# aksiksi/needle

Hardware: AMD Instinct MI355X
Metric: episode-pairs/sec (analyze+search) (higher is better)
Workload: dtype f64-certified (f32 first pass)

## Files before the change

include/needle_hip.h:

```cpp
#ifndef NEEDLE_HIP_H
#define NEEDLE_HIP_H

#include "needle.h"

#ifdef __cplusplus
extern "C" {
#endif

enum NeedleError needle_hip_device_count(int *count);
enum NeedleError needle_hip_set_device(int ordinal);
enum NeedleError needle_hip_synchronize(void);
enum NeedleError needle_hip_device_pci_bus_id(char out[32]);
void *needle_hip_stream(void);
const char *needle_hip_last_error_message(void);
const char *needle_hip_version(void);

enum NeedleError needle_hip_malloc(void **device_ptr, size_t bytes);
enum NeedleError needle_hip_free(void *device_ptr);
enum NeedleError needle_hip_memcpy_h2d(void *device_dst, const void *host_src, size_t bytes);
enum NeedleError needle_hip_memcpy_d2h(void *host_dst, const void *device_src, size_t bytes);
void needle_hip_host_free(void *ptr);
enum NeedleError needle_hip_host_alloc(void **host_ptr, size_t bytes);
enum NeedleError needle_hip_host_alloc_free(void *host_ptr);

double needle_hip_last_kernel_ms(const char *kernel);
void needle_hip_set_kernel_timing(const char *kernels);
enum NeedleError needle_hip_int_valu_ceiling(double *cells_per_second);
enum NeedleError needle_hip_scan_issued_evaluations(uint64_t *lane_evaluations, bool reset);
enum NeedleError needle_hip_scan_counts(uint64_t counts[2], bool reset);
enum NeedleError needle_hip_scan_last_launch(int32_t *form, uint64_t *matrix_products);
enum NeedleError needle_hip_epilogue_host_fallbacks(uint64_t *jobs, bool reset);

#define NEEDLE_HIP_MAX_CHANNELS 8
int needle_hip_fingerprint_sample_rate(void);
int needle_hip_fingerprint_delay_ms(void);
int needle_hip_fingerprint_item_duration_ms(void);
size_t needle_hip_fingerprint_num_items(size_t samples_per_channel);
size_t needle_hip_fingerprint_num_kept(size_t samples_per_channel, uint32_t step);

enum NeedleError needle_hip_fingerprint_host(const int16_t *const *pcm, const size_t *num_values,
                                             size_t num_streams, int channels, uint32_t step,
                                             uint32_t *const *items);

enum NeedleError needle_hip_fingerprint_device(const int16_t *d_pcm, const uint64_t *pcm_offsets,
                                               const uint64_t *num_values, size_t num_streams,
                                               int channels, uint32_t step, uint32_t *d_items,
                                               const uint64_t *item_offsets, bool sync);

enum NeedleError needle_hip_fingerprint_cert_stats(uint64_t counts[4], bool reset);

typedef struct NeedleHipCertAudit {
  uint64_t items, accepted, accepted_mismatches, mismatches;
  double max_error_over_s, max_s;
// ... 238 lines not shown
```

needle_amd/capi.py:

```python
from __future__ import annotations

import ctypes as C
import os
from dataclasses import dataclass
from typing import List, Optional, Sequence, Tuple

import numpy as np

NS = 1_000_000_000
LIB_PATH = os.environ.get("NEEDLE_CAPI_LIB") or os.path.join(os.path.dirname(os.path.abspath(__file__)), "lib", "libneedle_capi.so")

ERROR_NAMES = ["Ok", "InvalidUtf8String", "NullArgument", "InvalidArgument", "FrameHashDataNotFound",
               "FrameHashDataInvalidVersion", "InvalidFrameHashData", "ComparatorMinimumPaths",
               "AnalyzerInvalidHashPeriod", "AnalyzerInvalidHashDuration", "IOError", "Unknown"]

DEFAULT_HASH_MATCH_THRESHOLD = 10
DEFAULT_OPENING_SEARCH_PERCENTAGE = 0.50
DEFAULT_ENDING_SEARCH_PERCENTAGE = 0.25
DEFAULT_MIN_OPENING_DURATION = 20
DEFAULT_MIN_ENDING_DURATION = 20
DEFAULT_HASH_DURATION = 0.3
MAX_CHANNELS = 8


# ... 42 lines not shown
    "needle_hip_fingerprint_delay_ms", "needle_hip_fingerprint_item_duration_ms", "needle_hip_fingerprint_num_items",
    "needle_hip_fingerprint_num_kept", "needle_hip_fingerprint_host", "needle_hip_fingerprint_device",
    "needle_hip_fingerprint_debug", "needle_hip_resample_out_len", "needle_hip_resample_host", "needle_hip_downmix_host",
    "needle_hip_hamming_runs_device", "needle_hip_hamming_runs_host",
    "needle_hip_frame_hashes_new", "needle_hip_frame_hashes_free", "needle_hip_frame_hashes_len",
    "needle_hip_frame_hashes_copy", "needle_hip_frame_hashes_hash_duration_ns", "needle_hip_frame_hashes_md5",
    "needle_hip_frame_hashes_read", "needle_hip_frame_hashes_write", "needle_hip_header_md5",
    "needle_hip_analyzer_run_pcm", "needle_hip_comparator_run_with_frame_hashes", "needle_hip_library_new",
    "needle_hip_library_free", "needle_hip_library_include_endings", "needle_hip_library_set_sample_rate",
    "needle_hip_library_rows_per_video",
    "needle_hip_library_set_pcm", "needle_hip_library_set_pcm_device", "needle_hip_library_rank_videos",
    "needle_hip_library_analyze",
    "needle_hip_library_hash_arena", "needle_hip_library_use_hash_arena", "needle_hip_library_num_pairs", "needle_hip_library_search",
    "needle_hip_library_fetch_runs_begin", "needle_hip_library_fetch_runs_end",
    "needle_hip_library_finalize", "needle_hip_library_frame_hashes",
    "needle_hip_comm_create_id", "needle_hip_comm_init", "needle_hip_comm_finalize", "needle_hip_comm_rank",
    "needle_hip_comm_world_size", "needle_hip_comm_backend", "needle_hip_comm_barrier",
    "needle_hip_comm_all_gather_host", "needle_hip_comm_shard", "needle_hip_library_job_begin",
    "needle_hip_library_job_end", "needle_hip_library_stream_pcm", "needle_hip_host_alloc",
    "needle_hip_host_alloc_free", "needle_hip_int_valu_ceiling",
    "needle_hip_comparator_results_from_runs", "needle_hip_library_job_runs", "needle_hip_library_job_comm_bytes",
    "needle_hip_library_job_form",
    "needle_hip_host_threads", "needle_hip_fingerprint_audit_device", "needle_hip_library_audit",
    "needle_hip_scan_counts", "needle_hip_scan_last_launch", "needle_hip_epilogue_host_fallbacks",
    "needle_hip_index_new", "needle_hip_index_free", "needle_hip_index_len", "needle_hip_index_add",
    "needle_hip_index_results", "needle_hip_index_pairs_searched", "needle_hip_index_remove", "needle_hip_index_replace",
    "needle_hip_index_store_sizes", "needle_hip_index_crossmatcher_new", "needle_hip_index_add_matched",
    "needle_hip_index_pairs_scanned",
    "needle_hip_convert_host", "needle_hip_analyzer_run_pcm_format", "needle_hip_library_set_sample_format",
    "needle_hip_feeder_new", "needle_hip_feeder_free", "needle_hip_feeder_feed", "needle_hip_feeder_finish",
    "needle_hip_feeder_reset", "needle_hip_feeder_ready", "needle_hip_feeder_items", "needle_hip_feeder_frame_hashes",
    "needle_hip_feeder_state_bytes", "needle_hip_feeder_num_ready", "needle_hip_feeder_set_audit", "needle_hip_feeder_audit",
    "needle_hip_matcher_new", "needle_hip_matcher_free", "needle_hip_matcher_feed", "needle_hip_matcher_feed_from_feeder",
    "needle_hip_matcher_finish", "needle_hip_matcher_reset", "needle_hip_matcher_ready", "needle_hip_matcher_runs",
    "needle_hip_matcher_open", "needle_hip_matcher_stats",
    "needle_hip_crossmatcher_new", "needle_hip_crossmatcher_free", "needle_hip_crossmatcher_feed",
    "needle_hip_crossmatcher_feed_from_feeder", "needle_hip_crossmatcher_finish", "needle_hip_crossmatcher_ready",
    "needle_hip_crossmatcher_lane", "needle_hip_crossmatcher_runs", "needle_hip_crossmatcher_stats",
    "needle_hip_crossmatcher_state_bytes", "needle_hip_crossmatcher_new_regions",
    "needle_hip_crossmatcher_state_bytes_regions", "needle_hip_crossmatcher_shape",
    "needle_hip_crossmatcher_new_resident", "needle_hip_crossmatcher_state_bytes_resident", "needle_hip_crossmatcher_resident"]

SAMPLE_U8, SAMPLE_S16, SAMPLE_S32, SAMPLE_F32, SAMPLE_F64 = 0, 1, 2, 3, 4
SAMPLE_U8P, SAMPLE_S16P, SAMPLE_S32P, SAMPLE_F32P, SAMPLE_F64P = 5, 6, 7, 8, 9
_SAMPLE_DTYPES = [np.uint8, np.int16, np.int32, np.float32, np.float64]


# ... 246 lines not shown


def scan_issued_evaluations(reset: bool = False) -> int:
    v = C.c_uint64(0)
    lib().needle_hip_scan_issued_evaluations.argtypes = [C.POINTER(C.c_uint64), C.c_bool]
    check(lib().needle_hip_scan_issued_evaluations(C.byref(v), reset))
    return int(v.value)


def scan_counts(reset: bool = False) -> Tuple[int, int]:
    c = (C.c_uint64 * 2)()
    lib().needle_hip_scan_counts.argtypes = [C.POINTER(C.c_uint64), C.c_bool]
    check(lib().needle_hip_scan_counts(c, reset))
    return int(c[0]), int(c[1])


def scan_last_launch() -> Tuple[int, int]:
    form, products = C.c_int32(0), C.c_uint64(0)
    lib().needle_hip_scan_last_launch.argtypes = [C.POINTER(C.c_int32), C.POINTER(C.c_uint64)]
    check(lib().needle_hip_scan_last_launch(C.byref(form), C.byref(products)))
    return int(form.value), int(products.value)


def epilogue_host_fallbacks(reset: bool = False) -> int:
    jobs = C.c_uint64(0)
    lib().needle_hip_epilogue_host_fallbacks.argtypes = [C.POINTER(C.c_uint64), C.c_bool]
    check(lib().needle_hip_epilogue_host_fallbacks(C.byref(jobs), reset))
    return int(jobs.value)


def host_threads() -> int:
    lib().needle_hip_host_threads.restype = C.c_int
    return int(lib().needle_hip_host_threads())


def int_valu_ceiling() -> float:
    v = C.c_double(0.0)
    lib().needle_hip_int_valu_ceiling.argtypes = [C.POINTER(C.c_double)]
    check(lib().needle_hip_int_valu_ceiling(C.byref(v)))
    return v.value


def last_kernel_ms(name: str) -> float:
    return lib().needle_hip_last_kernel_ms(name.encode())


# ... 925 lines not shown
```

needle_amd/csrc/capi.cpp:

```cpp
#include <dirent.h>
#include <hip/hip_runtime_api.h>
#include <sys/stat.h>

#include <algorithm>
#include <cstdio>
#include <cstdlib>
#include <chrono>
#include <cstring>
#include <fstream>
#include <new>

#include "crossmatch.h"
#include "epilogue.h"
#include "hipctx.h"
#include "feeder.h"
#include "index.h"
#include "matcher.h"
#include "needle_core.h"

using namespace needle;

struct FrameHashes {
  FrameHashesData d;
};
// ... 409 lines not shown

enum NeedleError needle_hip_scan_issued_evaluations(uint64_t *lane_evaluations, bool reset) {
  if (!lane_evaluations) return NeedleError_NullArgument;
  return guarded([&]() -> NeedleError {
    Status s = gpu_scan_issued_evaluations(lane_evaluations, reset);
    return s.ok() ? NeedleError_Ok : report(s);
  });
}

enum NeedleError needle_hip_scan_counts(uint64_t counts[2], bool reset) {
  if (!counts) return NeedleError_NullArgument;
  return guarded([&]() -> NeedleError {
    Status s = gpu_scan_issued_evaluations(&counts[0], reset, &counts[1]);
    return s.ok() ? NeedleError_Ok : report(s);
  });
}

enum NeedleError needle_hip_scan_last_launch(int32_t *form, uint64_t *matrix_products) {
  if (!form || !matrix_products) return NeedleError_NullArgument;
  gpu_scan_last_launch(form, matrix_products);
  return NeedleError_Ok;
}

enum NeedleError needle_hip_epilogue_host_fallbacks(uint64_t *jobs, bool reset) {
  if (!jobs) return NeedleError_NullArgument;
  *jobs = reset ? epilogue_host_fallbacks().exchange(0) : epilogue_host_fallbacks().load();
  return NeedleError_Ok;
}

enum NeedleError needle_hip_int_valu_ceiling(double *cells_per_second) {
  if (!cells_per_second) return NeedleError_NullArgument;
  return guarded([&]() -> NeedleError {
    Status s = gpu_int_valu_ceiling(cells_per_second);
    return s.ok() ? NeedleError_Ok : report(s);
  });
}

double needle_hip_last_kernel_ms(const char *kernel) { return kernel ? kernel_ms(kernel) : -1.0; }
void needle_hip_set_kernel_timing(const char *kernels) { set_kernel_timing(kernels); }

int needle_hip_fingerprint_sample_rate(void) { return kSampleRate; }
int needle_hip_fingerprint_delay_ms(void) { return kDelayMs; }
int needle_hip_fingerprint_item_duration_ms(void) { return kItemDurationMs; }
size_t needle_hip_fingerprint_num_items(size_t samples_per_channel) { return num_items(samples_per_channel); }
size_t needle_hip_fingerprint_num_kept(size_t samples_per_channel, uint32_t step) {
  return num_kept(samples_per_channel, step);
// ... 771 lines not shown
```

needle_amd/csrc/common.h:

```cpp
#pragma once

#include <cstddef>
#include <cstdint>
#include <functional>
#include <string>
#include <vector>

#include "../../include/needle_hip.h"

struct ihipStream_t;

namespace needle {

struct Status {
  NeedleError code = NeedleError_Ok;
  std::string message;
  bool ok() const { return code == NeedleError_Ok; }
  static Status Ok() { return Status{}; }
  static Status Make(NeedleError c, std::string m) { return Status{c, std::move(m)}; }
};

NeedleError report(const Status &s);
void set_last_error(const std::string &m);
const char *last_error();
// ... 80 lines not shown
                              uint32_t step, uint32_t *d_items, bool sync, double *d_chroma_dbg = nullptr,
                              double *d_feat_dbg = nullptr, size_t descriptor_slot = 0, int pipe = -1,
                              uint32_t *zero_word = nullptr, bool *zeroed = nullptr);
Status gpu_fingerprint_streamed_device(const std::vector<const int16_t *> &pcm, const std::vector<size_t> &num_values,
                                       int channels, uint32_t step, uint32_t *d_items,
                                       const std::vector<uint64_t> &item_off, int rate = kSampleRate);
Status gpu_fingerprint_host(const std::vector<const int16_t *> &pcm, const std::vector<size_t> &num_values,
                            int channels, uint32_t step, std::vector<std::vector<uint32_t>> *items,
                            int rate = kSampleRate);
using PcmReader = std::function<Status(size_t stream, uint64_t first_value, uint64_t num_values, int16_t *dst)>;
using StreamIssued = std::function<Status(size_t stream_index)>;
Status gpu_upload_pcm_streamed(const std::vector<size_t> &num_values, const std::vector<uint64_t> &dev_off,
                               const PcmReader &read, unsigned readers, int16_t *d_pcm, ::ihipStream_t *stream = nullptr,
                               const StreamIssued &issued = nullptr);
Status gpu_upload_pcm(const std::vector<const int16_t *> &pcm, const std::vector<size_t> &num_values,
                      const std::vector<uint64_t> &dev_off, int16_t *d_pcm, ::ihipStream_t *stream = nullptr,
                      const StreamIssued &issued = nullptr);
Status gpu_fingerprint_streamed(const std::vector<size_t> &num_values, const PcmReader &read, unsigned readers,
                                int channels, uint32_t step, std::vector<std::vector<uint32_t>> *items,
                                int rate = kSampleRate);
Status gpu_hamming_runs_device(const uint32_t *d_hashes, const NeedleHipSeq *seqs, size_t num_seqs,
                               const NeedleHipProblem *problems, size_t num_problems, uint32_t threshold,
                               NeedleHipRun *d_runs, uint32_t capacity, uint32_t *d_count, bool sync,
                               bool count_is_zero = false);
Status gpu_hamming_runs_host(const uint32_t *hashes, size_t num_hashes, const NeedleHipSeq *seqs, size_t num_seqs,
                             const NeedleHipProblem *problems, size_t num_problems, uint32_t threshold,
                             std::vector<NeedleHipRun> *runs);

uint32_t *gpu_pinned_arena_acquire(size_t words);
void gpu_pinned_arena_release(uint32_t *arena);
void gpu_prefetch_hashes(const uint32_t *hashes, size_t num_hashes);

constexpr uint64_t kDeviceEpiloguePairs = 1u << 14;
constexpr uint32_t kDeviceEpilogueRuns = 1u << 14;

Status gpu_int_valu_ceiling(double *cells_per_second);
Status gpu_scan_issued_evaluations(uint64_t *lane_evaluations, bool reset, uint64_t *head_survivors = nullptr);
void gpu_scan_last_launch(int32_t *form, uint64_t *matrix_products);
Status gpu_fingerprint_cert_stats(uint64_t out[4], bool reset);
Status gpu_fingerprint_audit_device(const int16_t *d_pcm, const std::vector<StreamSpan> &spans, int channels, uint32_t step,
                                    const uint32_t *d_items, uint64_t out[4], double *max_ratio, double *max_sigma);

struct FeedLane {
  uint64_t pcm_off;
  uint64_t item_off;
  uint32_t row_base;
  uint32_t carried;
  uint32_t frames;
  uint32_t first_item;
  uint32_t kept;
  uint32_t lane;
};
constexpr size_t kFeedAuditWords = 6;
struct FeedAudit {
  double *rows64;
  uint64_t *counts;
};
Status gpu_fingerprint_feed_device(const int16_t *d_pcm, const std::vector<FeedLane> &lanes, int channels, uint32_t step,
                                   double *d_chroma, float *d_energy, double *d_chroma64, uint32_t *d_items,
                                   const FeedAudit *audit = nullptr);
bool gpu_fingerprint_f64_mode();
// ... 57 lines not shown
```

needle_amd/csrc/library.cpp:

```cpp
#include <hip/hip_runtime_api.h>

#include <algorithm>
#include <chrono>
#include <cstdio>
#include <cstdlib>
#include <cstring>
#include <map>
#include <new>
#include <tuple>

#include "comm.h"
#include "epilogue.h"
#include "hipctx.h"
#include "needle_core.h"

struct FrameHashes;
struct NeedleAudioComparator;

namespace needle {
const Comparator &comparator_of(const NeedleAudioComparator *c);
FrameHashes *make_frame_hashes(FrameHashesData &&d);
void fill_c_result(const VideoResult &v, NeedleHipSearchResult *r);
}

// ... 729 lines not shown
      if (num_pairs) pair_at(lib->n, first_pair, &i, &j);
      for (size_t p = first_pair; p < first_pair + num_pairs; p++) {
        for (size_t r = 0; r < Rc; r++) {
          if (r == 1 && (lib->win[i * R + 1].kept == 0 || lib->win[j * R + 1].kept == 0))
            return report(Status::Make(NeedleError_Unknown, "no ending hash data present"));
          const uint32_t a = lib->min_len[i * R + r], b = lib->min_len[j * R + r];
          if (a == 0 || b == 0) continue;
          problems.push_back(NeedleHipProblem{(uint32_t)(i * R + r), (uint32_t)(j * R + r), std::max(a, b),
                                              (uint32_t)(p * Rc + r)});
        }
        if (++j == lib->n) j = ++i + 1;
      }
      lib->problems_for[0] = first_pair;
      lib->problems_for[1] = num_pairs;
      lib->problems_for[2] = Rc;
    }
    for (NeedleHipLibrary::Fetch &f : lib->fetch)
      if (f.pending && (f.d_runs == d_runs || f.d_count == d_count) &&
          hipStreamWaitEvent(library_stream(), f.done, 0) != hipSuccess)
        return report(Status::Make(NeedleError_Unknown, "stream wait failed"));
    const auto t_built = std::chrono::steady_clock::now();
    const bool count_is_zero = lib->count_zeroed == d_count;
    lib->count_zeroed = nullptr;
    Status s = gpu_hamming_runs_device(lib->arena, seqs.data(), seqs.size(), problems.data(), problems.size(),
                                       cmp.hash_match_threshold(), d_runs, capacity, d_count, sync, count_is_zero);
    if (getenv("NEEDLE_HIP_TRACE"))
      std::fprintf(stderr, "[needle_hip] search enqueue: %zu problems built in %.2f ms, launched in %.2f ms\n",
                   problems.size(), std::chrono::duration<double, std::milli>(t_built - t_enter).count(),
                   std::chrono::duration<double, std::milli>(std::chrono::steady_clock::now() - t_built).count());
    return s.ok() ? NeedleError_Ok : report(s);
  });
}

enum NeedleError needle_hip_library_fetch_runs_begin(NeedleHipLibrary *lib, int slot, const NeedleHipRun *d_runs,
                                                     const uint32_t *d_count, uint32_t max_runs) {
  if (!lib || !d_runs || !d_count) return NeedleError_NullArgument;
  if (slot < 0 || slot > 1 || max_runs == 0) return NeedleError_InvalidArgument;
  return guarded([&]() -> NeedleError {
    NeedleHipLibrary::Fetch &f = lib->fetch[slot];
    if (f.pending) return report(Status::Make(NeedleError_InvalidArgument, "fetch slot still pending"));
    const size_t bytes = 16 + (size_t)max_runs * sizeof(NeedleHipRun);
    if (f.max_runs < max_runs) {
      if (f.host) (void)hipHostFree(f.host);
      f.host = nullptr;
      if (hipHostMalloc(&f.host, bytes, hipHostMallocDefault) != hipSuccess)
        return report(Status::Make(NeedleError_Unknown, "pinned allocation failed"));
      f.max_runs = max_runs;
    }
// ... 736 lines not shown
```

needle_amd/csrc/search.hip:

```cpp
#include "epilogue.h"
#include "hipctx.h"
#include "simhash_wave.h"

#include <algorithm>
#include <atomic>
#include <cstdio>
#include <cstdlib>
#include <cstring>
#include <mutex>
#include <unordered_map>

namespace needle {

namespace {

constexpr int kDiagsPerBlock = 256;
constexpr int kBandR = 7, kBandU = 3;
constexpr int kBandB = 64 * kBandR;
constexpr int kSampleW = 8;
constexpr int kSampleHead = 3;
__host__ __device__ constexpr int head_row(int k, int W, int H = kSampleHead) {
  return H == 3 ? (k == 0 ? 0 : (k == 1 ? W / 2 : W - 1)) : (k * (W - 1)) / (H - 1);
}
__host__ __device__ constexpr bool is_head_row(int s, int W, int H = kSampleHead) {
// ... 158 lines not shown
#pragma unroll
    for (int r = 0; r < R; r++) any |= (i + K - 1 - Z[r] >= flag_len);
    if (__any(any)) checkpoint(i + K - 1);
  }
  for (; i <= i_end; i++) {
    const uint32_t sv = src[i];
#pragma unroll
    for (int r = 0; r < R; r++) {
      const uint32_t c = (uint32_t)__popc(sv ^ W[r]);
      Z[r] = (c <= threshold) ? Z[r] : i;
    }
#pragma unroll
    for (int r = 0; r + 1 < R; r++) W[r] = W[r + 1];
    W[R - 1] = lds[B + i + d_l + R];
  }
}

__device__ __forceinline__ void wave_lds_fence_search() {
  __builtin_amdgcn_fence(__ATOMIC_RELEASE, "wavefront");
  __builtin_amdgcn_wave_barrier();
  __builtin_amdgcn_fence(__ATOMIC_ACQUIRE, "wavefront");
}

template <int R, int W, bool COUNT = false, int H = kSampleHead, bool LEGACY = false>
__global__ __launch_bounds__(256) void hamming_runs_sampled_kernel(const uint32_t *__restrict__ hashes,
                                                                   const SearchProblem *__restrict__ problems,
                                                                   int num_problems, uint32_t threshold,
                                                                   NeedleHipRun *__restrict__ runs,
                                                                   uint32_t capacity, uint32_t *__restrict__ count,
                                                                   int bands_per_wave, int sparse_max,
                                                                   unsigned long long *__restrict__ eval_groups) {
  constexpr int B = 64 * R;
  unsigned long long groups = 0, survived = 0;
  extern __shared__ uint32_t lds[];
  __builtin_amdgcn_s_setprio(3);
  int lo = 0, hi = num_problems - 1;
  while (lo < hi) {
    int mid = (lo + hi + 1) >> 1;
    if (problems[mid].block_base <= blockIdx.x) lo = mid; else hi = mid - 1;
  }
  const SearchProblem pr = problems[lo];
  const int n = (int)pr.n, m = (int)pr.m;
  const uint32_t *__restrict__ src = hashes + pr.src_off;
  const uint32_t *__restrict__ dst = hashes + pr.dst_off;
  uint32_t *ldst = lds;
  for (int k = threadIdx.x; k < B; k += blockDim.x) {
    ldst[k] = 0u;
    ldst[B + m + k] = 0u;
  }
  {
    constexpr int kU = 8;
    const int nt = (int)blockDim.x;
    int k = threadIdx.x;
    for (; k + (kU - 1) * nt < m; k += kU * nt) {
// ... 46 lines not shown

  int k0 = (i_start - 1 + P - 1) / P;
  for (int w0 = 1 + k0 * P; w0 + W - 1 <= i_end; w0 += P) {
    uint32_t E[W + R - 1];
#pragma unroll
    for (int q = 0; q < W + R - 1; q++) E[q] = ldst[B + w0 + d_l + q];
    uint32_t sv[W];
#pragma unroll
    for (int s = 0; s < W; s++) sv[s] = src[w0 + s];
    bool ok[R];
    uint32_t miss[R];
#pragma unroll
    for (int r = 0; r < R; r++) miss[r] = 0u;
#pragma unroll
    for (int k = 0; k < H; k++) {
      const int s = head_row(k, W, H);
#pragma unroll
      for (int r = 0; r < R; r++) miss[r] |= (uint32_t)__popc(sv[s] ^ E[s + r]) + bias;
    }
#pragma unroll
    for (int r = 0; r < R; r++) ok[r] = miss[r] < 32u;
    if (COUNT) groups += H * R;
    auto resolve = [&](const int d) {
      const int ilo = d < 0 ? 1 - d : 1;
      const int ihi = min(n - 1, m - 1 - d);
      if (w0 < ilo || w0 + W - 1 > ihi) return;
      int e = w0 + W;
      bool ended = false;
      const int fwd_limit = min(ihi, w0 + P + W - 1);
      while (e <= fwd_limit) {
        const int row = e + lane;
        const bool bad = row <= fwd_limit && (uint32_t)__popc(lsrc[row] ^ ldst[B + row + d]) > threshold;
        if (COUNT) groups += 1;
        const unsigned long long mm = __ballot(bad);
        if (mm) {
          e += __ffsll((long long)mm) - 1;
          ended = true;
          break;
        }
        e += 64;
      }
      if (!ended) {
        if (fwd_limit == w0 + P + W - 1) return;
        e = ihi + 1;
      }
      const int b = e - 1;
      int a = ilo;
      int q = w0 - 1;
      while (q >= ilo) {
        const int row = q - lane;
        const bool bad = row >= ilo && (uint32_t)__popc(lsrc[row] ^ ldst[B + row + d]) > threshold;
        if (COUNT) groups += 1;
        const unsigned long long mm = __ballot(bad);
        if (mm) {
          a = q - (__ffsll((long long)mm) - 1) + 1;
          break;
        }
        q -= 64;
      }
      const int len = b - a + 1;
      if (len >= min_len) emit_run((uint32_t)b, (uint32_t)(b + d), (uint32_t)len);
    };

    unsigned long long alive[R];
    int survivors = 0;
#pragma unroll
    for (int r = 0; r < R; r++) {
      alive[r] = __ballot(ok[r]);
      survivors += __popcll(alive[r]);
    }
    if (COUNT) survived += (unsigned long long)survivors;
    if (survivors == 0) continue;
    if (!LEGACY || sparse_max < 0) {
#pragma unroll
      for (int r = 0; r < R; r++) {
        if (alive[r] == 0) continue;
        uint32_t mm = miss[r];
#pragma unroll
        for (int k = 0; k < W - H; k++) {
          const int s = tail_row(k, W, H);
          mm |= (uint32_t)__popc(sv[s] ^ E[s + r]) + bias;
        }
        if (COUNT) groups += W - H;
        unsigned long long cand = __ballot(mm < 32u);
        while (cand) {
          const int src_lane = __ffsll((long long)cand) - 1;
          cand &= cand - 1;
          resolve(D0 + src_lane * R + r);
        }
      }
      continue;
    }
    if constexpr (LEGACY) {
    if (survivors <= sparse_max) {
      constexpr int kTail = W - H;
      uint32_t sv_tail = sv[tail_row(kTail - 1, W, H)];
      int tail_off = tail_row(kTail - 1, W, H);
#pragma unroll
      for (int k = kTail - 2; k >= 0; k--) {
        sv_tail = lane == k ? sv[tail_row(k, W, H)] : sv_tail;
        tail_off = lane == k ? tail_row(k, W, H) : tail_off;
      }
#pragma unroll
      for (int r = 0; r < R; r++) {
        unsigned long long cand = alive[r];
        while (cand) {
          const int src_lane = __ffsll((long long)cand) - 1;
// ... 13 lines not shown
#pragma unroll
      for (int r = 0; r < R; r++) miss[r] |= (uint32_t)__popc(sv[s] ^ E[s + r]) + bias;
    }
#pragma unroll
    for (int r = 0; r < R; r++) ok[r] = miss[r] < 32u;
    if (COUNT) groups += (W - H) * R;
#pragma unroll
    for (int r = 0; r < R; r++) {
      unsigned long long cand = __ballot(ok[r]);
      while (cand) {
        const int src_lane = __ffsll((long long)cand) - 1;
        cand &= cand - 1;
        resolve(D0 + src_lane * R + r);
      }
    }
    }
  }
  }
  flush_runs();
  if (COUNT && lane == 0) {
    atomicAdd(eval_groups, groups);
    atomicAdd(eval_groups + 1, survived);
  }
}

__host__ __device__ constexpr int mfma_windows(int n, int min_len, int W) {
  return (n - 1 - W) >= 0 && min_len - W + 1 > 0 ? (n - 1 - W) / (min_len - W + 1) + 1 : 0;
}
typedef int mfma_v4i __attribute__((ext_vector_type(4)));
typedef int mfma_v8i __attribute__((ext_vector_type(8)));
typedef float mfma_v16f __attribute__((ext_vector_type(16)));

#include "scan_mfma_kernel.h"


__global__ __launch_bounds__(256) void simhash_runs_kernel(const uint32_t *__restrict__ hashes,
                                                           const SearchProblem *__restrict__ problems,
                                                           NeedleHipRun *__restrict__ runs, uint32_t capacity,
                                                           const uint32_t *__restrict__ count) {
  const uint32_t total = min(*count, capacity);
  const uint32_t wave = (blockIdx.x * blockDim.x + threadIdx.x) >> 6, waves = (gridDim.x * blockDim.x) >> 6;
  const uint32_t lane = threadIdx.x & 63;
  __builtin_amdgcn_s_setprio(3);
  const TransposeLane t = transpose_lane(lane);
  for (uint32_t k = wave; k < total; k += waves) {
    const NeedleHipRun r = runs[k];
// ... 3 lines not shown
    if (lane == 0) {
      runs[k].problem = pr.tag;
      runs[k].src_match_hash = src_hash;
      runs[k].dst_match_hash = dst_hash;
    }
  }
}

struct ScanShape {
  int w = kSampleW, h = kSampleHead;
};
ScanShape scan_shape() {
  ScanShape sh;
  if (const char *e = getenv("NEEDLE_HIP_SCAN_SHAPE")) {
    int w = 0, h = 0;
    if (std::sscanf(e, "%d,%d", &w, &h) == 2 && (w == 4 || w == 8 || w == 16) && h >= 2 && h <= 4 && h < w) {
      sh.w = w;
      sh.h = h;
    }
  }
  return sh;
}
using SampledKernel = void (*)(const uint32_t *, const SearchProblem *, int, uint32_t, NeedleHipRun *, uint32_t, uint32_t *, int, int,
                               unsigned long long *);
template <bool COUNT>
SampledKernel sampled_kernel(ScanShape sh, bool legacy) {
#define NEEDLE_SHAPE(W_, H_) \
  if (sh.w == W_ && sh.h == H_) return hamming_runs_sampled_kernel<kBandR, W_, COUNT, H_, true>;
  NEEDLE_SHAPE(4, 2) NEEDLE_SHAPE(4, 3) NEEDLE_SHAPE(8, 2) NEEDLE_SHAPE(8, 4) NEEDLE_SHAPE(16, 2) NEEDLE_SHAPE(16, 3) NEEDLE_SHAPE(16, 4)
#undef NEEDLE_SHAPE
  if (legacy) return hamming_runs_sampled_kernel<kBandR, kSampleW, COUNT, kSampleHead, true>;
  return hamming_runs_sampled_kernel<kBandR, kSampleW, COUNT, kSampleHead, false>;
}

struct SearchPlan {
  std::vector<NeedleHipSeq> seqs;
  std::vector<NeedleHipProblem> problems;
  int mode[8] = {0, 0, 0, 0, 0, 0, 0, 0};
  std::vector<SearchProblem> meta;
  size_t staged = 0;
  uint64_t oversize_blocks = 0;
  uint64_t blocks = 0;
  size_t lds_bytes = 0;
  bool sampled = false, fast = false, mfma = false;
  int mfma_waves = 0, mfma_splits = 1;
  std::vector<M2ImageSeq> image_seqs;
  uint32_t image_windows = 0, image_min_len = 0;
// ... 217 lines not shown
}

int mfma_request(uint32_t threshold) {
  if (threshold > 15u || scan_shape().w != kSampleW || getenv("NEEDLE_HIP_SCAN_SHAPE") || getenv("NEEDLE_HIP_SCAN_COUNT")) return 0;
  const char *e = getenv("NEEDLE_HIP_SCAN_MFMA");
  if (!e) return 2;
  return atoi(e) != 0 ? 1 : 0;
}

int mfma_waves() {
  int waves = 8;
  if (const char *e = getenv("NEEDLE_HIP_MFMA_WAVES")) {
    const int w = atoi(e);
    if (w == 4 || w == 8 || w == 12 || w == 16) waves = w;
  }
  return waves;
}
using Mfma2Kernel = void (*)(const uint32_t *, const SearchProblem *, int, uint32_t, NeedleHipRun *, uint32_t, uint32_t *, int, const uint32_t *);
Mfma2Kernel mfma2_kernel(int waves) {
  return waves == 4 ? hamming_runs_mfma2_kernel<kSampleW, 4, 3> : waves == 16 ? hamming_runs_mfma2_kernel<kSampleW, 16, 4>
       : waves == 12 ? hamming_runs_mfma2_kernel<kSampleW, 12, 3> : hamming_runs_mfma2_kernel<kSampleW, 8, 4>;
}

std::atomic<int32_t> g_last_form{0};
std::atomic<uint64_t> g_last_products{0};

struct SearchWorkspace {
  DeviceBuffer<SearchProblem> problems;
  PinnedStage stage;
  DescriptorUpload<SearchProblem> upload;
  SearchPlan plan;
  DeviceBuffer<M2ImageSeq> image_seqs;
  PinnedStage image_stage;
  DescriptorUpload<M2ImageSeq> image_upload;
  DeviceBuffer<uint32_t> images;
  bool lds_attr_set = false;
  unsigned long long *eval_groups = nullptr;
};
std::mutex g_ws_mu;
std::map<int, SearchWorkspace *> g_ws;

SearchWorkspace *workspace() {
  int dev = 0;
  (void)hipGetDevice(&dev);
  std::lock_guard<std::mutex> lock(g_ws_mu);
  auto it = g_ws.find(dev);
  if (it != g_ws.end()) return it->second;
  SearchWorkspace *w = new SearchWorkspace();
  g_ws[dev] = w;
  return w;
}


}

void gpu_scan_last_launch(int32_t *form, uint64_t *matrix_products) {
  *form = g_last_form.load();
  *matrix_products = g_last_products.load();
}

Status gpu_hamming_runs_device(const uint32_t *d_hashes, const NeedleHipSeq *seqs, size_t num_seqs,
                               const NeedleHipProblem *problems, size_t num_problems, uint32_t threshold,
                               NeedleHipRun *d_runs, uint32_t capacity, uint32_t *d_count, bool sync, bool count_is_zero) {
  std::lock_guard<std::recursive_mutex> gpu_lock(gpu_mutex());
  Status s = ensure_device();
  if (!s.ok()) return s;
  hipStream_t stream = library_stream();
  if (!count_is_zero) NEEDLE_HIP_TRY(hipMemsetAsync(d_count, 0, sizeof(uint32_t), stream));
  const int mode[8] = {getenv("NEEDLE_HIP_GENERIC_SEARCH") != nullptr, getenv("NEEDLE_HIP_BAND_SEARCH") != nullptr,
                       getenv("NEEDLE_HIP_BANDS_PER_WAVE") ? std::max(1, atoi(getenv("NEEDLE_HIP_BANDS_PER_WAVE"))) : 0,
                       threshold > 31u,
                       mfma_request(threshold),
                       getenv("NEEDLE_HIP_SEARCH_LDS_LIMIT") ? std::max(1, atoi(getenv("NEEDLE_HIP_SEARCH_LDS_LIMIT"))) : 160 * 1024,
                       mfma_waves(),
                       (getenv("NEEDLE_HIP_MFMA_SPLITS") ? std::max(1, std::min(64, atoi(getenv("NEEDLE_HIP_MFMA_SPLITS")))) : 0) |
                           (getenv("NEEDLE_HIP_MFMA_SINGLE") ? 0x100 : 0) | (getenv("NEEDLE_HIP_MFMA_NO_IMAGES") ? 0x200 : 0)};
  SearchWorkspace *ws = workspace();
  SearchPlan &plan = ws->plan;
  const bool reuse = plan.matches(seqs, num_seqs, problems, num_problems, mode);
  if (!reuse && !(s = build_plan(seqs, num_seqs, problems, num_problems, mode, &plan)).ok()) return s;
  const std::vector<SearchProblem> &meta = plan.meta;
  const uint64_t blocks = plan.blocks;
  const size_t lds_bytes = plan.lds_bytes;
  const bool sampled = plan.sampled, fast = plan.fast;
  const int bands_per_wave = plan.bands_per_wave;
  if (!meta.empty()) {
    if (!(reuse && ws->upload.resident_at == ws->problems.ptr && ws->problems.ptr) &&
        !(s = ws->upload.put(&ws->problems, &ws->stage, meta, stream)).ok())
      return s;
    if (lds_bytes > 64 * 1024 && !ws->lds_attr_set) {
      NEEDLE_HIP_TRY(hipFuncSetAttribute(reinterpret_cast<const void *>(hamming_runs_kernel<true>),
                                         hipFuncAttributeMaxDynamicSharedMemorySize, 160 * 1024));
      NEEDLE_HIP_TRY(hipFuncSetAttribute(reinterpret_cast<const void *>(hamming_runs_band_kernel<kBandR, kBandU>),
                                         hipFuncAttributeMaxDynamicSharedMemorySize, 160 * 1024));
      for (int w : {4, 8, 12, 16})
        NEEDLE_HIP_TRY(hipFuncSetAttribute(reinterpret_cast<const void *>(mfma2_kernel(w)),
                                           hipFuncAttributeMaxDynamicSharedMemorySize, 160 * 1024));
      for (int w : {4, 8, 16})
        for (int h : {2, 3, 4}) {
          if (h >= w) continue;
          for (bool legacy : {false, true}) {
            NEEDLE_HIP_TRY(hipFuncSetAttribute(reinterpret_cast<const void *>(sampled_kernel<false>(ScanShape{w, h}, legacy)),
                                               hipFuncAttributeMaxDynamicSharedMemorySize, 160 * 1024));
            NEEDLE_HIP_TRY(hipFuncSetAttribute(reinterpret_cast<const void *>(sampled_kernel<true>(ScanShape{w, h}, legacy)),
                                               hipFuncAttributeMaxDynamicSharedMemorySize, 160 * 1024));
          }
        }
      ws->lds_attr_set = true;
    }
    const int staged = (int)plan.staged, oversize = (int)(meta.size() - plan.staged);
    g_last_form.store(staged > 0 ? (sampled ? (plan.mfma ? 4 : 3) : fast ? 2 : 1) : 1);
    g_last_products.store(staged > 0 && plan.mfma ? plan.mfma_products : 0);
    if (staged > 0) {
      KernelTimer timer("hamming_runs");
      if (sampled) {
        int sparse_max = -1;
        if (const char *e = getenv("NEEDLE_HIP_SPARSE_MAX")) sparse_max = std::max(0, atoi(e));
        if (getenv("NEEDLE_HIP_SCAN_COUNT")) {
          if (!ws->eval_groups) {
            NEEDLE_HIP_TRY(hipMalloc((void **)&ws->eval_groups, 2 * sizeof(unsigned long long)));
            NEEDLE_HIP_TRY(hipMemsetAsync(ws->eval_groups, 0, 2 * sizeof(unsigned long long), stream));
          }
          hipLaunchKernelGGL(sampled_kernel<true>(scan_shape(), sparse_max >= 0), dim3((uint32_t)blocks), dim3(256), lds_bytes, stream, d_hashes,
                             ws->problems.ptr, staged, threshold, d_runs, capacity, d_count, bands_per_wave, sparse_max,
                             ws->eval_groups);
        } else if (plan.mfma) {
          const uint32_t *images = nullptr;
          if (!plan.image_seqs.empty()) {
            if (!(s = ws->image_upload.put(&ws->image_seqs, &ws->image_stage, plan.image_seqs, stream)).ok() ||
                !(s = ws->images.reserve((size_t)plan.image_windows * kM2ImageWords)).ok())
              return s;
            const uint32_t grid = (uint32_t)std::min<uint64_t>(8192, ((uint64_t)plan.image_windows * kM2Rows + 255) / 256);
            hipLaunchKernelGGL(m2_window_images_kernel<kSampleW>, dim3(grid), dim3(256), 0, stream, d_hashes, ws->image_seqs.ptr,
                               (int)plan.image_seqs.size(), plan.image_windows, plan.image_min_len, ws->images.ptr);
            images = ws->images.ptr;
          }
          hipLaunchKernelGGL(mfma2_kernel(plan.mfma_waves), dim3((uint32_t)blocks), dim3(64 * plan.mfma_waves),
                             lds_bytes, stream, d_hashes, ws->problems.ptr, staged, threshold, d_runs, capacity, d_count,
                             plan.mfma_splits, images);
#if NEEDLE_M2_LAB & 8
          {
            unsigned long long c[8], z[8] = {};
            (void)hipStreamSynchronize(stream);
            (void)hipMemcpyFromSymbol(c, HIP_SYMBOL(m2_dbg), sizeof c);
            (void)hipMemcpyToSymbol(HIP_SYMBOL(m2_dbg), z, sizeof z);
            fprintf(stderr, "m2 counts: resolve calls %llu, trips %llu, mismatches handled %llu, walks continued %llu, extra forward trips %llu, "
                            "windows past the tail rows %llu, items %llu, windows past the head rows %llu\n", c[0], c[1], c[2], c[3], c[4], c[5], c[6], c[7]);
          }
#endif
        } else {
          hipLaunchKernelGGL(sampled_kernel<false>(scan_shape(), sparse_max >= 0), dim3((uint32_t)blocks), dim3(256), lds_bytes, stream, d_hashes,
                             ws->problems.ptr, staged, threshold, d_runs, capacity, d_count, bands_per_wave, sparse_max,
                             (unsigned long long *)nullptr);
        }
      }
      else if (fast)
        hipLaunchKernelGGL((hamming_runs_band_kernel<kBandR, kBandU>), dim3((uint32_t)blocks), dim3(256), lds_bytes,
                           stream, d_hashes, ws->problems.ptr, staged, threshold, d_runs, capacity, d_count);
      else
        hipLaunchKernelGGL(hamming_runs_kernel<true>, dim3((uint32_t)blocks), dim3(256), lds_bytes, stream, d_hashes,
                           ws->problems.ptr, staged, 0u, threshold, d_runs, capacity, d_count);
    }
    if (oversize > 0) {
      KernelTimer timer("hamming_runs_unstaged");
      hipLaunchKernelGGL(hamming_runs_kernel<false>, dim3((uint32_t)plan.oversize_blocks), dim3(256), 0, stream, d_hashes,
                         ws->problems.ptr + staged, oversize, (uint32_t)staged, threshold, d_runs, capacity, d_count);
    }
    {
      KernelTimer timer("simhash_runs");
      hipLaunchKernelGGL(simhash_runs_kernel, dim3(2048), dim3(256), 0, stream, d_hashes, ws->problems.ptr, d_runs,
                         capacity, d_count);
    }
    NEEDLE_HIP_TRY(hipGetLastError());
  }
  if (sync) NEEDLE_HIP_TRY(hipStreamSynchronize(stream));
  return Status::Ok();
}

Status gpu_scan_issued_evaluations(uint64_t *lane_evaluations, bool reset, uint64_t *head_survivors) {
  std::lock_guard<std::recursive_mutex> gpu_lock(gpu_mutex());
  Status s = ensure_device();
  if (!s.ok()) return s;
  SearchWorkspace *ws = workspace();
  unsigned long long groups[2] = {0, 0};
  hipStream_t stream = library_stream();
  if (ws->eval_groups) {
    NEEDLE_HIP_TRY(hipMemcpyAsync(groups, ws->eval_groups, sizeof(groups), hipMemcpyDeviceToHost, stream));
    if (reset) NEEDLE_HIP_TRY(hipMemsetAsync(ws->eval_groups, 0, sizeof(groups), stream));
    NEEDLE_HIP_TRY(hipStreamSynchronize(stream));
  }
  *lane_evaluations = (uint64_t)groups[0] * 64u;
  if (head_survivors) *head_survivors = (uint64_t)groups[1];
  return Status::Ok();
}

namespace {
struct HostCallBuffers {
  DeviceBuffer<uint32_t> d_hashes, d_count;
// ... 265 lines not shown
```

rust/needle-hip/src/ffi.rs:

```rust
#![allow(non_camel_case_types, dead_code)]

use std::os::raw::{c_char, c_int, c_void};

#[repr(C)]
#[derive(Clone, Copy, Debug, PartialEq, Eq)]
pub enum NeedleError {
    Ok = 0,
    InvalidUtf8String,
    NullArgument,
    InvalidArgument,
    FrameHashDataNotFound,
    FrameHashDataInvalidVersion,
    InvalidFrameHashData,
    ComparatorMinimumPaths,
    AnalyzerInvalidHashPeriod,
    AnalyzerInvalidHashDuration,
    IOError,
    Unknown,
}

#[repr(C)]
pub struct NeedleAudioAnalyzer {
    _private: [u8; 0],
}
// ... 101 lines not shown
        min_opening_duration: u16,
        min_ending_duration: u16,
        time_padding: f32,
        output: *mut *const NeedleAudioComparator,
    ) -> NeedleError;
    pub fn needle_audio_comparator_free(comparator: *const NeedleAudioComparator);
    pub fn needle_audio_comparator_run(
        comparator: *const NeedleAudioComparator,
        analyze: bool,
        display: bool,
        use_skip_files: bool,
        write_skip_files: bool,
        threading: bool,
    ) -> NeedleError;

    pub fn needle_hip_last_error_message() -> *const c_char;
    pub fn needle_hip_device_count(count: *mut c_int) -> NeedleError;
    pub fn needle_hip_set_device(ordinal: c_int) -> NeedleError;
    pub fn needle_hip_synchronize() -> NeedleError;
    pub fn needle_hip_device_pci_bus_id(out: *mut c_char) -> NeedleError;
    pub fn needle_hip_fingerprint_cert_stats(counts: *mut u64, reset: bool) -> NeedleError;
    pub fn needle_hip_scan_issued_evaluations(lane_evaluations: *mut u64, reset: bool) -> NeedleError;
    pub fn needle_hip_scan_last_launch(form: *mut i32, matrix_products: *mut u64) -> NeedleError;
    pub fn needle_hip_epilogue_host_fallbacks(jobs: *mut u64, reset: bool) -> NeedleError;
    pub fn needle_hip_stream() -> *mut c_void;
    pub fn needle_hip_analyzer_run_pcm(
        analyzer: *mut NeedleAudioAnalyzer,
        pcm: *const *const i16,
        num_values: *const usize,
        channels: c_int,
        sample_rate: c_int,
        hash_duration: f32,
        persist: bool,
    ) -> NeedleError;
    pub fn needle_hip_analyzer_run_pcm_format(
        analyzer: *mut NeedleAudioAnalyzer,
        pcm: *const *const c_void,
        num_values: *const usize,
        channels: c_int,
        sample_rate: c_int,
        format: c_int,
        hash_duration: f32,
        persist: bool,
    ) -> NeedleError;
    pub fn needle_hip_comparator_run_with_frame_hashes(
        comparator: *const NeedleAudioComparator,
// ... 262 lines not shown
```

Before: 702,500.

## Defer crowded candidate groups from the sampled scan to a load-balanced second kernel

When a wave's sampled scan finds many candidate diagonals at once (at least eight), it now writes a compact crowd record instead of resolving them serially, and a follow-up kernel splits each record across several waves, reading hashes from global memory. The goal is to remove the tail latency that a few heavily matching waves impose on the main scan. The path is enabled only when the previous search returned many runs per problem, or when an environment variable forces it. It adds a second launch, a global-memory resolve path, and bounded record capacity with parity-swapped counters.

```diff
diff --git a/include/needle_hip.h b/include/needle_hip.h
--- a/include/needle_hip.h
+++ b/include/needle_hip.h
@@ -29,6 +29,7 @@
 enum NeedleError needle_hip_scan_issued_evaluations(uint64_t *lane_evaluations, bool reset);
 enum NeedleError needle_hip_scan_counts(uint64_t counts[2], bool reset);
 enum NeedleError needle_hip_scan_last_launch(int32_t *form, uint64_t *matrix_products);
+enum NeedleError needle_hip_scan_deferred(uint64_t *records, uint64_t *candidates, int reset);
 enum NeedleError needle_hip_epilogue_host_fallbacks(uint64_t *jobs, bool reset);
 
 #define NEEDLE_HIP_MAX_CHANNELS 8
diff --git a/needle_amd/capi.py b/needle_amd/capi.py
--- a/needle_amd/capi.py
+++ b/needle_amd/capi.py
@@ -88,7 +88,7 @@
     "needle_hip_comparator_results_from_runs", "needle_hip_library_job_runs", "needle_hip_library_job_comm_bytes",
     "needle_hip_library_job_form",
     "needle_hip_host_threads", "needle_hip_fingerprint_audit_device", "needle_hip_library_audit",
-    "needle_hip_scan_counts", "needle_hip_scan_last_launch", "needle_hip_epilogue_host_fallbacks",
+    "needle_hip_scan_counts", "needle_hip_scan_last_launch", "needle_hip_scan_deferred", "needle_hip_epilogue_host_fallbacks",
     "needle_hip_index_new", "needle_hip_index_free", "needle_hip_index_len", "needle_hip_index_add",
     "needle_hip_index_results", "needle_hip_index_pairs_searched", "needle_hip_index_remove", "needle_hip_index_replace",
     "needle_hip_index_store_sizes", "needle_hip_index_crossmatcher_new", "needle_hip_index_add_matched",
@@ -381,6 +381,13 @@
     return int(form.value), int(products.value)
 
 
+def scan_deferred(reset: bool = False) -> Tuple[int, int]:
+    records, candidates = C.c_uint64(0), C.c_uint64(0)
+    lib().needle_hip_scan_deferred.argtypes = [C.POINTER(C.c_uint64), C.POINTER(C.c_uint64), C.c_int]
+    check(lib().needle_hip_scan_deferred(C.byref(records), C.byref(candidates), int(reset)))
+    return int(records.value), int(candidates.value)
+
+
 def epilogue_host_fallbacks(reset: bool = False) -> int:
     jobs = C.c_uint64(0)
     lib().needle_hip_epilogue_host_fallbacks.argtypes = [C.POINTER(C.c_uint64), C.c_bool]
diff --git a/needle_amd/csrc/capi.cpp b/needle_amd/csrc/capi.cpp
--- a/needle_amd/csrc/capi.cpp
+++ b/needle_amd/csrc/capi.cpp
@@ -455,6 +455,14 @@
   return NeedleError_Ok;
 }
 
+enum NeedleError needle_hip_scan_deferred(uint64_t *records, uint64_t *candidates, int reset) {
+  if (!records || !candidates) return NeedleError_NullArgument;
+  return guarded([&]() -> NeedleError {
+    Status s = gpu_scan_deferred(records, candidates, reset != 0);
+    return s.ok() ? NeedleError_Ok : report(s);
+  });
+}
+
 enum NeedleError needle_hip_epilogue_host_fallbacks(uint64_t *jobs, bool reset) {
   if (!jobs) return NeedleError_NullArgument;
   *jobs = reset ? epilogue_host_fallbacks().exchange(0) : epilogue_host_fallbacks().load();
diff --git a/needle_amd/csrc/common.h b/needle_amd/csrc/common.h
--- a/needle_amd/csrc/common.h
+++ b/needle_amd/csrc/common.h
@@ -126,7 +126,7 @@
 Status gpu_hamming_runs_device(const uint32_t *d_hashes, const NeedleHipSeq *seqs, size_t num_seqs,
                                const NeedleHipProblem *problems, size_t num_problems, uint32_t threshold,
                                NeedleHipRun *d_runs, uint32_t capacity, uint32_t *d_count, bool sync,
-                               bool count_is_zero = false);
+                               bool count_is_zero = false, bool crowds_expected = false);
 Status gpu_hamming_runs_host(const uint32_t *hashes, size_t num_hashes, const NeedleHipSeq *seqs, size_t num_seqs,
                              const NeedleHipProblem *problems, size_t num_problems, uint32_t threshold,
                              std::vector<NeedleHipRun> *runs);
@@ -137,10 +137,12 @@
 
 constexpr uint64_t kDeviceEpiloguePairs = 1u << 14;
 constexpr uint32_t kDeviceEpilogueRuns = 1u << 14;
+constexpr uint64_t kCrowdRunsPerProblem = 8;
 
 Status gpu_int_valu_ceiling(double *cells_per_second);
 Status gpu_scan_issued_evaluations(uint64_t *lane_evaluations, bool reset, uint64_t *head_survivors = nullptr);
 void gpu_scan_last_launch(int32_t *form, uint64_t *matrix_products);
+Status gpu_scan_deferred(uint64_t *records, uint64_t *candidates, bool reset);
 Status gpu_fingerprint_cert_stats(uint64_t out[4], bool reset);
 Status gpu_fingerprint_audit_device(const int16_t *d_pcm, const std::vector<StreamSpan> &spans, int channels, uint32_t step,
                                     const uint32_t *d_items, uint64_t out[4], double *max_ratio, double *max_sigma);
diff --git a/needle_amd/csrc/library.cpp b/needle_amd/csrc/library.cpp
--- a/needle_amd/csrc/library.cpp
+++ b/needle_amd/csrc/library.cpp
@@ -775,8 +775,9 @@
     const auto t_built = std::chrono::steady_clock::now();
     const bool count_is_zero = lib->count_zeroed == d_count;
     lib->count_zeroed = nullptr;
+    const bool crowds_expected = lib->last_max_count > 0 && (uint64_t)lib->last_max_count >= kCrowdRunsPerProblem * (uint64_t)problems.size();
     Status s = gpu_hamming_runs_device(lib->arena, seqs.data(), seqs.size(), problems.data(), problems.size(),
-                                       cmp.hash_match_threshold(), d_runs, capacity, d_count, sync, count_is_zero);
+                                       cmp.hash_match_threshold(), d_runs, capacity, d_count, sync, count_is_zero, crowds_expected);
     if (getenv("NEEDLE_HIP_TRACE"))
       std::fprintf(stderr, "[needle_hip] search enqueue: %zu problems built in %.2f ms, launched in %.2f ms\n",
                    problems.size(), std::chrono::duration<double, std::milli>(t_built - t_enter).count(),
diff --git a/needle_amd/csrc/search.hip b/needle_amd/csrc/search.hip
--- a/needle_amd/csrc/search.hip
+++ b/needle_amd/csrc/search.hip
@@ -204,14 +204,108 @@
   __builtin_amdgcn_fence(__ATOMIC_ACQUIRE, "wavefront");
 }
 
-template <int R, int W, bool COUNT = false, int H = kSampleHead, bool LEGACY = false>
+struct DstLds {
+  const uint32_t *ldst;
+  int pad;
+  static constexpr bool kEager = false;
+  __device__ __forceinline__ uint32_t operator()(int row, int d) const { return ldst[pad + row + d]; }
+};
+struct DstGlobal {
+  const uint32_t *dst;
+  static constexpr bool kEager = true;
+  __device__ __forceinline__ uint32_t operator()(int row, int d) const { return dst[row + d]; }
+};
+template <int W, bool COUNT, class Dst>
+__device__ __forceinline__ bool resolve_candidate(const int d, const int w0, const int P, const int n, const int m, const int min_len,
+                                                  const uint32_t threshold, const int lane, const uint32_t *__restrict__ lsrc,
+                                                  const Dst dst, unsigned long long &groups, int *b_out, int *len_out) {
+  const int ilo = d < 0 ? 1 - d : 1;
+  const int ihi = min(n - 1, m - 1 - d);
+  if (w0 < ilo || w0 + W - 1 > ihi) return false;
+  int e = w0 + W;
+  bool ended = false;
+  const int fwd_limit = min(ihi, w0 + P + W - 1);
+  bool bad_f0 = false, bad_b0 = false;
+  if constexpr (Dst::kEager) {
+    const int rf = e + lane, rb = w0 - 1 - lane;
+    const bool vf = rf <= fwd_limit, vb = rb >= ilo;
+    uint32_t sf = 0u, df = 0u, sb = 0u, db = 0u;
+    if (vf) {
+      sf = lsrc[rf];
+      df = dst(rf, d);
+    }
+    if (vb) {
+      sb = lsrc[rb];
+      db = dst(rb, d);
+    }
+    bad_f0 = vf && (uint32_t)__popc(sf ^ df) > threshold;
+    bad_b0 = vb && (uint32_t)__popc(sb ^ db) > threshold;
+    if (COUNT) groups += 2;
+  }
+  while (e <= fwd_limit) {
+    const int row = e + lane;
+    bool bad;
+    if (Dst::kEager && e == w0 + W) {
+      bad = bad_f0;
+    } else {
+      bad = row <= fwd_limit && (uint32_t)__popc(lsrc[row] ^ dst(row, d)) > threshold;
+      if (COUNT) groups += 1;
+    }
+    const unsigned long long mm = __ballot(bad);
+    if (mm) {
+      e += __ffsll((long long)mm) - 1;
+      ended = true;
+      break;
+    }
+    e += 64;
+  }
+  if (!ended) {
+    if (fwd_limit == w0 + P + W - 1) return false;
+    e = ihi + 1;
+  }
+  const int b = e - 1;
+  int a = ilo;
+  int q = w0 - 1;
+  while (q >= ilo) {
+    const int row = q - lane;
+    bool bad;
+    if (Dst::kEager && q == w0 - 1) {
+      bad = bad_b0;
+    } else {
+      bad = row >= ilo && (uint32_t)__popc(lsrc[row] ^ dst(row, d)) > threshold;
+      if (COUNT) groups += 1;
+    }
+    const unsigned long long mm = __ballot(bad);
+    if (mm) {
+      a = q - (__ffsll((long long)mm) - 1) + 1;
+      break;
+    }
+    q -= 64;
+  }
+  const int len = b - a + 1;
+  *b_out = b;
+  *len_out = len;
+  return len >= min_len;
+}
+
+struct CrowdRecord {
+  uint32_t entry;
+  int32_t w0, d0;
+  uint32_t pad;
+  unsigned long long mask;
+};
+constexpr int kCrowdSplit = 8;
+
+template <int R, int W, bool COUNT = false, int H = kSampleHead, bool LEGACY = false, bool DEFER = false>
 __global__ __launch_bounds__(256) void hamming_runs_sampled_kernel(const uint32_t *__restrict__ hashes,
                                                                    const SearchProblem *__restrict__ problems,
                                                                    int num_problems, uint32_t threshold,
                                                                    NeedleHipRun *__restrict__ runs,
                                                                    uint32_t capacity, uint32_t *__restrict__ count,
                                                                    int bands_per_wave, int sparse_max,
-                                                                   unsigned long long *__restrict__ eval_groups) {
+                                                                   unsigned long long *__restrict__ eval_groups,
+                                                                   CrowdRecord *__restrict__ crowds, uint32_t *__restrict__ crowd_count,
+                                                                   uint32_t crowd_capacity, uint32_t defer_from) {
   constexpr int B = 64 * R;
   unsigned long long groups = 0, survived = 0;
   extern __shared__ uint32_t lds[];
@@ -304,44 +398,9 @@
     for (int r = 0; r < R; r++) ok[r] = miss[r] < 32u;
     if (COUNT) groups += H * R;
     auto resolve = [&](const int d) {
-      const int ilo = d < 0 ? 1 - d : 1;
-      const int ihi = min(n - 1, m - 1 - d);
-      if (w0 < ilo || w0 + W - 1 > ihi) return;
-      int e = w0 + W;
-      bool ended = false;
-      const int fwd_limit = min(ihi, w0 + P + W - 1);
-      while (e <= fwd_limit) {
-        const int row = e + lane;
-        const bool bad = row <= fwd_limit && (uint32_t)__popc(lsrc[row] ^ ldst[B + row + d]) > threshold;
-        if (COUNT) groups += 1;
-        const unsigned long long mm = __ballot(bad);
-        if (mm) {
-          e += __ffsll((long long)mm) - 1;
-          ended = true;
-          break;
-        }
-        e += 64;
-      }
-      if (!ended) {
-        if (fwd_limit == w0 + P + W - 1) return;
-        e = ihi + 1;
-      }
-      const int b = e - 1;
-      int a = ilo;
-      int q = w0 - 1;
-      while (q >= ilo) {
-        const int row = q - lane;
-        const bool bad = row >= ilo && (uint32_t)__popc(lsrc[row] ^ ldst[B + row + d]) > threshold;
-        if (COUNT) groups += 1;
-        const unsigned long long mm = __ballot(bad);
-        if (mm) {
-          a = q - (__ffsll((long long)mm) - 1) + 1;
-          break;
-        }
-        q -= 64;
-      }
-      const int len = b - a + 1;
-      if (len >= min_len) emit_run((uint32_t)b, (uint32_t)(b + d), (uint32_t)len);
+      int b, len;
+      if (resolve_candidate<W, COUNT>(d, w0, P, n, m, min_len, threshold, lane, lsrc, DstLds{ldst, B}, groups, &b, &len))
+        emit_run((uint32_t)b, (uint32_t)(b + d), (uint32_t)len);
     };
 
     unsigned long long alive[R];
@@ -365,6 +424,17 @@
         }
         if (COUNT) groups += W - H;
         unsigned long long cand = __ballot(mm < 32u);
+        if constexpr (DEFER) {
+          if ((uint32_t)__popcll(cand) >= defer_from) {
+            uint32_t slot = 0u;
+            if (lane == 0) slot = atomicAdd(crowd_count, 1u);
+            slot = (uint32_t)__builtin_amdgcn_readfirstlane((int)slot);
+            if (slot < crowd_capacity) {
+              if (lane == 0) crowds[slot] = CrowdRecord{(uint32_t)lo, w0, D0 + r, 0u, cand};
+              cand = 0ull;
+            }
+          }
+        }
         while (cand) {
           const int src_lane = __ffsll((long long)cand) - 1;
           cand &= cand - 1;
@@ -424,6 +494,71 @@
     atomicAdd(eval_groups, groups);
     atomicAdd(eval_groups + 1, survived);
   }
+}
+
+template <int R, int W>
+__global__ __launch_bounds__(256) void hamming_crowds_kernel(const uint32_t *__restrict__ hashes,
+                                                             const SearchProblem *__restrict__ problems, uint32_t threshold,
+                                                             NeedleHipRun *__restrict__ runs, uint32_t capacity,
+                                                             uint32_t *__restrict__ count,
+                                                             const CrowdRecord *__restrict__ crowds, uint32_t crowd_capacity,
+                                                             uint32_t *__restrict__ counters, int parity) {
+  __builtin_amdgcn_s_setprio(3);
+  const uint32_t records = min(counters[parity], crowd_capacity);
+  const int lane = (int)(threadIdx.x & 63);
+  if (blockIdx.x == 0) {
+    unsigned long long *totals = reinterpret_cast<unsigned long long *>(counters + 2);
+    uint32_t c = 0u;
+    for (uint32_t k = threadIdx.x; k < records; k += blockDim.x) c += (uint32_t)__popcll(crowds[k].mask);
+    for (int step = 32; step >= 1; step >>= 1) c += (uint32_t)__shfl_xor((int)c, step);
+    if (lane == 0 && c) atomicAdd(totals + 1, (unsigned long long)c);
+    if (threadIdx.x == 0) {
+      counters[parity ^ 1] = 0u;
+      if (records) atomicAdd(totals, (unsigned long long)records);
+    }
+  }
+  if (records == 0u) return;
+  const uint32_t wave = (uint32_t)__builtin_amdgcn_readfirstlane((int)((blockIdx.x * blockDim.x + threadIdx.x) >> 6));
+  const uint32_t waves = (gridDim.x * blockDim.x) >> 6;
+  uint32_t held_entry = 0u, held_b = 0u, held_e = 0u, held_len = 0u;
+  int held = 0;
+  auto flush_runs = [&]() {
+    if (held == 0) return;
+    uint32_t base = 0u;
+    if (lane == 0) base = atomicAdd(count, (uint32_t)held);
+    base = (uint32_t)__builtin_amdgcn_readfirstlane((int)base);
+    if (lane < held && base + (uint32_t)lane < capacity)
+      runs[base + (uint32_t)lane] = NeedleHipRun{held_entry, held_b, held_e, held_len, 0u, 0u};
+    held = 0;
+  };
+  unsigned long long groups = 0;
+  const uint32_t items = records * (uint32_t)kCrowdSplit;
+  for (uint32_t item = wave; item < items; item += waves) {
+    const CrowdRecord rec = crowds[item / (uint32_t)kCrowdSplit];
+    const int share = (int)(item % (uint32_t)kCrowdSplit);
+    const SearchProblem pr = problems[rec.entry];
+    const int n = (int)pr.n, m = (int)pr.m, min_len = (int)pr.min_len;
+    const int P = min_len - W + 1;
+    const uint32_t *__restrict__ src = hashes + pr.src_off;
+    const DstGlobal dst{hashes + pr.dst_off};
+    unsigned long long cand = rec.mask;
+    for (int rank = 0; cand; rank++) {
+      const int src_lane = __ffsll((long long)cand) - 1;
+      cand &= cand - 1;
+      if (rank % kCrowdSplit != share) continue;
+      const int d = rec.d0 + src_lane * R;
+      int b, len;
+      if (resolve_candidate<W, false>(d, rec.w0, P, n, m, min_len, threshold, lane, src, dst, groups, &b, &len)) {
+        const bool mine = lane == held;
+        held_entry = mine ? rec.entry : held_entry;
+        held_b = mine ? (uint32_t)b : held_b;
+        held_e = mine ? (uint32_t)(b + d) : held_e;
+        held_len = mine ? (uint32_t)len : held_len;
+        if (++held == 64) flush_runs();
+      }
+    }
+  }
+  flush_runs();
 }
 
 __host__ __device__ constexpr int mfma_windows(int n, int min_len, int W) {
@@ -473,7 +608,9 @@
   return sh;
 }
 using SampledKernel = void (*)(const uint32_t *, const SearchProblem *, int, uint32_t, NeedleHipRun *, uint32_t, uint32_t *, int, int,
-                               unsigned long long *);
+                               unsigned long long *, CrowdRecord *, uint32_t *, uint32_t, uint32_t);
+SampledKernel deferring_kernel() { return hamming_runs_sampled_kernel<kBandR, kSampleW, false, kSampleHead, false, true>; }
+bool deferring_shape(ScanShape sh) { return sh.w == kSampleW && sh.h == kSampleHead; }
 template <bool COUNT>
 SampledKernel sampled_kernel(ScanShape sh, bool legacy) {
 #define NEEDLE_SHAPE(W_, H_) \
@@ -737,6 +874,13 @@
        : waves == 12 ? hamming_runs_mfma2_kernel<kSampleW, 12, 3> : hamming_runs_mfma2_kernel<kSampleW, 8, 4>;
 }
 
+constexpr uint32_t kDeferFrom = 8, kCrowdCapacity = 1u << 16;
+constexpr int kCrowdBlocksPerCu = 4;
+bool defer_request(bool hint) {
+  if (const char *e = getenv("NEEDLE_HIP_SCAN_DEFER")) return atoi(e) != 0;
+  return hint;
+}
+
 std::atomic<int32_t> g_last_form{0};
 std::atomic<uint64_t> g_last_products{0};
 
@@ -751,6 +895,9 @@
   DeviceBuffer<uint32_t> images;
   bool lds_attr_set = false;
   unsigned long long *eval_groups = nullptr;
+  DeviceBuffer<CrowdRecord> crowds;
+  uint32_t *crowd_counters = nullptr;
+  int crowd_parity = 0;
 };
 std::mutex g_ws_mu;
 std::map<int, SearchWorkspace *> g_ws;
@@ -776,7 +923,8 @@
 
 Status gpu_hamming_runs_device(const uint32_t *d_hashes, const NeedleHipSeq *seqs, size_t num_seqs,
                                const NeedleHipProblem *problems, size_t num_problems, uint32_t threshold,
-                               NeedleHipRun *d_runs, uint32_t capacity, uint32_t *d_count, bool sync, bool count_is_zero) {
+                               NeedleHipRun *d_runs, uint32_t capacity, uint32_t *d_count, bool sync, bool count_is_zero,
+                               bool crowds_expected) {
   std::lock_guard<std::recursive_mutex> gpu_lock(gpu_mutex());
   Status s = ensure_device();
   if (!s.ok()) return s;
@@ -821,6 +969,8 @@
                                                hipFuncAttributeMaxDynamicSharedMemorySize, 160 * 1024));
           }
         }
+      NEEDLE_HIP_TRY(hipFuncSetAttribute(reinterpret_cast<const void *>(deferring_kernel()),
+                                         hipFuncAttributeMaxDynamicSharedMemorySize, 160 * 1024));
       ws->lds_attr_set = true;
     }
     const int staged = (int)plan.staged, oversize = (int)(meta.size() - plan.staged);
@@ -838,7 +988,7 @@
           }
           hipLaunchKernelGGL(sampled_kernel<true>(scan_shape(), sparse_max >= 0), dim3((uint32_t)blocks), dim3(256), lds_bytes, stream, d_hashes,
                              ws->problems.ptr, staged, threshold, d_runs, capacity, d_count, bands_per_wave, sparse_max,
-                             ws->eval_groups);
+                             ws->eval_groups, (CrowdRecord *)nullptr, (uint32_t *)nullptr, 0u, 0u);
         } else if (plan.mfma) {
           const uint32_t *images = nullptr;
           if (!plan.image_seqs.empty()) {
@@ -863,10 +1013,27 @@
                             "windows past the tail rows %llu, items %llu, windows past the head rows %llu\n", c[0], c[1], c[2], c[3], c[4], c[5], c[6], c[7]);
           }
 #endif
+        } else if (defer_request(crowds_expected) && sparse_max < 0 && deferring_shape(scan_shape())) {
+          uint32_t defer_from = kDeferFrom, crowd_capacity = kCrowdCapacity;
+          if (const char *e = getenv("NEEDLE_HIP_SCAN_DEFER_FROM")) defer_from = (uint32_t)std::max(1, std::min(65, atoi(e)));
+          if (const char *e = getenv("NEEDLE_HIP_SCAN_DEFER_CAP")) crowd_capacity = (uint32_t)std::max(1, std::min(1 << 24, atoi(e)));
+          if (!(s = ws->crowds.reserve(crowd_capacity)).ok()) return s;
+          if (!ws->crowd_counters) {
+            NEEDLE_HIP_TRY(hipMalloc((void **)&ws->crowd_counters, 8 * sizeof(uint32_t)));
+            NEEDLE_HIP_TRY(hipMemsetAsync(ws->crowd_counters, 0, 8 * sizeof(uint32_t), stream));
+          }
+          const int parity = ws->crowd_parity;
+          ws->crowd_parity ^= 1;
+          hipLaunchKernelGGL(deferring_kernel(), dim3((uint32_t)blocks), dim3(256), lds_bytes, stream, d_hashes, ws->problems.ptr, staged,
+                             threshold, d_runs, capacity, d_count, bands_per_wave, sparse_max, (unsigned long long *)nullptr,
+                             ws->crowds.ptr, ws->crowd_counters + parity, crowd_capacity, defer_from);
+          hipLaunchKernelGGL((hamming_crowds_kernel<kBandR, kSampleW>), dim3((uint32_t)(kCrowdBlocksPerCu * device_cus())), dim3(256), 0, stream,
+                             d_hashes, ws->problems.ptr, threshold, d_runs, capacity, d_count, ws->crowds.ptr, crowd_capacity,
+                             ws->crowd_counters, parity);
         } else {
           hipLaunchKernelGGL(sampled_kernel<false>(scan_shape(), sparse_max >= 0), dim3((uint32_t)blocks), dim3(256), lds_bytes, stream, d_hashes,
                              ws->problems.ptr, staged, threshold, d_runs, capacity, d_count, bands_per_wave, sparse_max,
-                             (unsigned long long *)nullptr);
+                             (unsigned long long *)nullptr, (CrowdRecord *)nullptr, (uint32_t *)nullptr, 0u, 0u);
         }
       }
       else if (fast)
@@ -889,6 +1056,23 @@
     NEEDLE_HIP_TRY(hipGetLastError());
   }
   if (sync) NEEDLE_HIP_TRY(hipStreamSynchronize(stream));
+  return Status::Ok();
+}
+
+Status gpu_scan_deferred(uint64_t *records, uint64_t *candidates, bool reset) {
+  std::lock_guard<std::recursive_mutex> gpu_lock(gpu_mutex());
+  Status s = ensure_device();
+  if (!s.ok()) return s;
+  SearchWorkspace *ws = workspace();
+  unsigned long long totals[2] = {0, 0};
+  hipStream_t stream = library_stream();
+  if (ws->crowd_counters) {
+    NEEDLE_HIP_TRY(hipMemcpyAsync(totals, ws->crowd_counters + 2, sizeof(totals), hipMemcpyDeviceToHost, stream));
+    if (reset) NEEDLE_HIP_TRY(hipMemsetAsync(ws->crowd_counters + 2, 0, sizeof(totals), stream));
+    NEEDLE_HIP_TRY(hipStreamSynchronize(stream));
+  }
+  *records = (uint64_t)totals[0];
+  *candidates = (uint64_t)totals[1];
   return Status::Ok();
 }
 
diff --git a/rust/needle-hip/src/ffi.rs b/rust/needle-hip/src/ffi.rs
--- a/rust/needle-hip/src/ffi.rs
+++ b/rust/needle-hip/src/ffi.rs
@@ -147,6 +147,7 @@
     pub fn needle_hip_fingerprint_cert_stats(counts: *mut u64, reset: bool) -> NeedleError;
     pub fn needle_hip_scan_issued_evaluations(lane_evaluations: *mut u64, reset: bool) -> NeedleError;
     pub fn needle_hip_scan_last_launch(form: *mut i32, matrix_products: *mut u64) -> NeedleError;
+    pub fn needle_hip_scan_deferred(records: *mut u64, candidates: *mut u64, reset: c_int) -> NeedleError;
     pub fn needle_hip_epilogue_host_fallbacks(jobs: *mut u64, reset: bool) -> NeedleError;
     pub fn needle_hip_stream() -> *mut c_void;
     pub fn needle_hip_analyzer_run_pcm(
```

Result: slower. 691,000 (-1.6%).
